# kevinh-e/BetaOne

Hardware: AMD Instinct MI355X
Metric: mcts_nodes_per_sec (higher is better)
Workload: dtype f32 (3 x f16 split, f32 accumulate)

## Files before the change

betaone_amd/csrc/bo_engine.cpp:

```cpp
#include "../../include/betaone_engine.h"
#include "../../include/betaone_lab.h"

#include "bo_tree.h"
#include "bo_fastw.h"
#include "bo_select_wide.h"
#include "bo_replay.h"
#include "bo_train.h"
#include "bo_metrics.h"
#include "bo_pgn.h"
#include "bo_san.h"
#include "bo_analyse.h"
#include "bo_reanalyse.h"
#include "bo_perft.h"
#include "bo_mate.h"
#include "bo_book.h"
#include "bo_merge.h"
#include "bo_tb.h"
#include "bo_nn_fused.h"
#include "bo_conv.h"
#include "bo_tower.h"
#include "bo_tower_wg.h"
#include "bo_tower_h.h"
#include "bo_tower_s.h"
#include "bo_tower_s16.h"
// ... 31 lines not shown
    int sel_profile = 0, sel_pending = 0;
    long long sel_launches = 0;
    double sel_ms = 0.0;
#if !defined(BO_WAVE_EMU)
    hipEvent_t sel_ev0 = nullptr, sel_ev1 = nullptr;
#endif
    bool fast = false;
    bo_config cfg;
    int device;
    std::vector<void *> allocs;
    int *d_go = nullptr, *d_action = nullptr;
    std::vector<int> h_i32;
    std::vector<HostRng> rng;
    int *d_res_blk = nullptr, *d_info_blk = nullptr;
    int *h_res = nullptr, *h_info = nullptr;
    int watch_seen = 0;
    double *h_noise = nullptr;
    int *h_go = nullptr;
    int *h_action = nullptr;
    int action_flip = 0;
    rt_event ev_action[2]{};
    bool ev_action_made[2] = {false, false};
    bool ship = true;
    bool prefetch_valid = false;
    std::vector<int> h_nl, h_term;
    bool nl_valid = false;
    void *setup_dev = nullptr, *setup_host = nullptr;
    size_t setup_cap = 0;
    std::vector<unsigned char> noise_pending;
    std::vector<int> lazy_want;
    bool begin_lazy = false, ev_begin_made = false;
    rt_event ev_begin{};
    double *h_turn_u = nullptr;
    int *h_turn_flags = nullptr;
    double *d_turn_pw = nullptr;
    std::vector<double> turn_pw_host;
    double turn_pw_tfinal = 0.0;
    int *d_turn_action = nullptr, *d_turn_state = nullptr, *d_turn_cres = nullptr;
    float *d_turn_rv = nullptr;
    int *d_turn_resigned = nullptr, *d_turn_rnext = nullptr;
    std::vector<int> resign_en;
    float resign_t = 0.0f;
    int resign_k = 1;
    float *d_root_value = nullptr;
    TbTable *d_tb_tabs = nullptr;
    std::vector<int> turn_want;
// ... 146 lines not shown
    int **iscal[] = {&d.sims_done, &d.n_nodes, &d.rows, &d.n_runs, &d.n_ul, &d.req_nlegal, &d.status,
                     &d.trk_n, &d.n_hist, &d.ctx_mode, &d.root_nch, &d.stat_evals,
                     &d.stat_flushes, &d.stat_term_sims, &d.stat_levels, &d.stat_children_scanned, &e->d_go, &e->d_action};
    for (int **p : iscal) rc |= e->alloc(p, G);
    const size_t res_ints = G * (4 + 2 * (size_t)BO_RES_CAP) + 4, info_ints = G * 18;
    rc |= e->alloc(&e->d_res_blk, res_ints); rc |= e->alloc(&e->d_info_blk, info_ints);
    if (!rc) {
        d.res_n = e->d_res_blk; d.res_best_idx = e->d_res_blk + G; d.res_best_mv = e->d_res_blk + 2 * G; d.res_total = e->d_res_blk + 3 * G;
        d.res_idx = e->d_res_blk + 4 * G; d.res_val = reinterpret_cast<float *>(e->d_res_blk + 4 * G + G * BO_RES_CAP);
        d.res_watch = e->d_res_blk + G * (4 + 2 * (size_t)BO_RES_CAP); d.watch = nullptr; d.watch_n = 1;
        d.phase = e->d_info_blk; d.req_node = e->d_info_blk + G; d.root_nlegal = e->d_info_blk + 2 * G; d.root_term = e->d_info_blk + 3 * G;
        d.ply = e->d_info_blk + 4 * G;
        e->d_turn_action = e->d_info_blk + 5 * G; e->d_turn_state = e->d_info_blk + 6 * G; e->d_turn_cres = e->d_info_blk + 7 * G;
        e->d_turn_rv = reinterpret_cast<float *>(e->d_info_blk + 15 * G); e->d_turn_resigned = e->d_info_blk + 16 * G;
        e->d_turn_rnext = e->d_info_blk + 17 * G;
        rt_memset(e->d_res_blk, 0, res_ints * 4, nullptr); rt_memset(e->d_info_blk, 0, info_ints * 4, nullptr);
    }
    rc |= rt_host_alloc((void **)&e->h_res, res_ints * 4); rc |= rt_host_alloc((void **)&e->h_info, info_ints * 4);
    rc |= rt_host_alloc((void **)&e->h_noise, G * BO_MAX_MOVES * sizeof(double)); rc |= rt_host_alloc((void **)&e->h_go, G * 4);
    rc |= rt_host_alloc((void **)&e->h_action, 2 * G * 4);
    rc |= rt_host_alloc((void **)&e->h_turn_u, G * sizeof(double)); rc |= rt_host_alloc((void **)&e->h_turn_flags, G * 4);
    rc |= e->alloc(&e->d_turn_pw, (size_t)cfg->num_simulations + 1);
    { const char *v = getenv("BETAONE_TURN_COPIES"); e->ship = !(v && v[0] == '1'); }
    rc |= e->alloc(&d.gpos, G * c.PLY_CAP); rc |= e->alloc(&d.trk, G * c.TRK_CAP); rc |= e->alloc(&d.trk_cnt, G * c.TRK_CAP);
    rc |= e->alloc(&d.hist, G * 7);
    rc |= e->alloc(&d.n_visits, N); rc |= e->alloc(&d.parent, N); rc |= e->alloc(&d.first_child, N); rc |= e->alloc(&d.n_children, N);
    rc |= e->alloc(&d.q, N); rc |= e->alloc(&d.prior, N); rc |= e->alloc(&d.move, N); rc |= e->alloc(&d.term, N);
    rc |= e->alloc(&d.eval_slot, N); rc |= e->alloc(&d.npos, N);
    rc |= e->alloc(&d.run_leaf, G * c.B); rc |= e->alloc(&d.run_cnt, G * c.B);
    rc |= e->alloc(&d.ul_node, G * c.UL_MAX); rc |= e->alloc(&d.ul_nlegal, G * c.UL_MAX); rc |= e->alloc(&d.ul_value, G * c.UL_MAX);
    rc |= e->alloc(&d.ul_move, G * c.UL_MAX * BO_CH_CAP); rc |= e->alloc(&d.ul_prior, G * c.UL_MAX * BO_CH_CAP);
    rc |= e->alloc(&d.req_moves, G * BO_MAX_MOVES); rc |= e->alloc(&d.root_moves, G * BO_MAX_MOVES);
    rc |= e->alloc(&d.root_child_rank, G * 2 * BO_CH_CAP); rc |= e->alloc(&d.noise, G * BO_MAX_MOVES);
    rc |= e->alloc(&d.played, G * c.PLY_CAP);
    rc |= e->alloc(&d.prof, G * BO_PROF_SLOTS);
    rc |= e->alloc(&d.resign_cnt, 2 * G); rc |= e->alloc(&e->d_root_value, G);
    if (!rc) rt_memset(d.resign_cnt, 0, 2 * G * 4, nullptr);
    rc |= e->alloc(&e->d_tb_tabs, (size_t)TB_MAX_TABLES); rc |= e->alloc(&d.tb_stat, 3 * G);
    if (!rc) rt_memset(d.tb_stat, 0, 3 * G * 4, nullptr);
    d.tb_tabs = e->d_tb_tabs; d.tb_n = 0; d.tb_flags = 0;
    d.played_now = nullptr;
    if (fast) {
        FastW &f = e->f;
        const size_t L = (size_t)cfg->leaves_per_step;
        f.L = (int)L;
        f.sel_ut = 2; f.sel_flags = FW_SEL_OCT;
// ... 248 lines not shown
    e->prefetch_valid = false;
    if (e->fast) {
        const int rows = e->d.c.G * e->f.L;
        if (policy_kind != BO_POLICY_NONE) RT(RT_LAUNCH(bo_k_fw_apply, rows, stream, e->d, e->f, policy_dev, policy_kind));
#if !defined(BO_WAVE_EMU)
        if (e->sel_profile) {
            if (!e->sel_ev0) { RT((int)hipEventCreate(&e->sel_ev0)); RT((int)hipEventCreate(&e->sel_ev1)); }
            if (e->sel_pending) {
                float ms = 0.0f;
                RT((int)hipEventSynchronize(e->sel_ev1));
                RT((int)hipEventElapsedTime(&ms, e->sel_ev0, e->sel_ev1));
                e->sel_ms += ms; e->sel_launches++; e->sel_pending = 0;
            }
            RT((int)hipEventRecord(e->sel_ev0, (hipStream_t)stream));
        }
#endif
        RT(launch_fw_select(e, value_dev, policy_kind, stream));
#if !defined(BO_WAVE_EMU)
        if (e->sel_profile) { RT((int)hipEventRecord(e->sel_ev1, (hipStream_t)stream)); e->sel_pending = 1; }
#endif
        RT(RT_LAUNCH(bo_k_fw_leaf, rows, stream, e->d, e->f, nn_in_dev));
    } else {
        if (e->d.tb_n > 0 && (e->d.tb_flags & TBF_SEARCH)) RT(RT_LAUNCH(bo_k_step_tb, e->d.c.G, stream, e->d, policy_dev, value_dev, policy_kind, nn_in_dev, vt));
        else RT(RT_LAUNCH(bo_k_step, e->d.c.G, stream, e->d, policy_dev, value_dev, policy_kind, nn_in_dev, vt));
    }
    return BO_OK;
}
extern "C" int bo_step(bo_engine *e, const float *policy_dev, const float *value_dev, int policy_kind, float *nn_in_dev,
                       void *stream) {
    if (!e || !nn_in_dev) return fail(BO_E_ARG, "null argument");
    if (policy_kind != BO_POLICY_NONE && (!policy_dev || !value_dev)) return fail(BO_E_ARG, "policy/value required");
    return step_launch(e, policy_dev, value_dev, policy_kind, nn_in_dev, stream, StepTail{nullptr, nullptr, nullptr, nullptr, 0});
}
extern "C" int bo_step_heads(bo_engine *e, const float *logits_dev, const float *vpart_dev, const float *b1_dev, const float *w2_dev,
                             const float *b2_dev, int rows, float *nn_in_dev, void *stream) {
    if (!e || !nn_in_dev || !logits_dev || !vpart_dev || !b1_dev || !w2_dev || !b2_dev) return fail(BO_E_ARG, "null argument");
    if (e->fast) return fail(BO_E_CONFIG, "bo_step_heads: the reference-semantics search only (fast mode evaluates rows, not games)");
    if (rows < e->d.c.G) return fail(BO_E_ARG, "bo_step_heads: the partial sums must hold a row per game (rows >= G)");
    return step_launch(e, logits_dev, nullptr, BO_POLICY_LOGITS, nn_in_dev, stream, StepTail{vpart_dev, b1_dev, w2_dev, b2_dev, rows});
}

extern "C" int bo_search_poll(bo_engine *e, int32_t *n_running, int32_t *n_requested, int32_t *requested_mask, void *stream) {
    if (!e) return fail(BO_E_ARG, "null engine");
    const size_t G = (size_t)e->d.c.G;
    RT(rt_d2h(e->h_info, e->d_info_blk, 2 * G * 4, stream));
    const int *ph = e->h_info, *rq = e->h_info + G;
    RT(rt_sync(stream));
// ... 382 lines not shown
        RT(rt_h2d(e->d_turn_pw, e->turn_pw_host.data(), ((size_t)S + 1) * sizeof(double), stream));
        RT(rt_sync(stream));
        e->turn_pw_tfinal = t_final;
    }
    if (!redo) {
        for (int g = 0; g < G; g++) {
            const double temp = move_number[g] < threshold ? t_initial : t_final;
            int fl = (active[g] ? 1 : 0) | (want_next[g] ? 4 : 0);
            if (active[g] && !(fabs(temp - 1.0) < 1e-6)) fl |= 2;
            if (active[g] && (int)e->resign_en.size() == G && e->resign_en[g]) fl |= 8;
            e->h_turn_flags[g] = fl;
            if (active[g]) e->h_turn_u[g] = hr_double(&e->rng[g]);
        }
        e->turn_want.assign(want_next, want_next + G);
    }
    TurnArgs a;
    a.u = e->h_turn_u; a.flags = e->h_turn_flags; a.pw = e->d_turn_pw;
    a.action = e->d_turn_action; a.state = e->d_turn_state; a.cres = e->d_turn_cres;
    a.root_value = e->d_turn_rv; a.resigned = e->d_turn_resigned; a.resign_next = e->d_turn_rnext;
    a.resign_t = e->resign_t; a.resign_k = e->resign_k;
    e->prefetch_valid = false;
    e->nl_valid = false;
    RT(RT_LAUNCH(bo_k_turn_sample, G, stream, e->d, a));
    RT(RT_LAUNCH(bo_k_turn_play, G, stream, e->d, a, nn_in_dev));
    const size_t Gs = (size_t)G, watch_off = Gs * (4 + 2 * (size_t)BO_RES_CAP);
    int rc = ship(e, e->h_info + 2 * Gs, (const int *)e->d_info_blk + 2 * Gs, 15 * Gs, e->h_res + watch_off, (const int *)e->d_res_blk + watch_off, 4, stream);
    if (rc) return rc;
    if (!e->ev_turn_made) { RT(rt_event_create(&e->ev_turn)); e->ev_turn_made = true; }
    RT(rt_event_record(e->ev_turn, stream));
    rc = bo_step(e, nullptr, nullptr, BO_POLICY_NONE, nn_in_dev, stream);
    if (rc) return rc;
    e->turn_outstanding = true;
    return BO_OK;
}

extern "C" int bo_selfplay_autoturn_ready(bo_engine *e, int32_t *ready_out) {
    if (!e || !ready_out) return fail(BO_E_ARG, "null argument");
    if (!e->turn_outstanding) return fail(BO_E_STATE, "no bo_selfplay_autoturn outstanding");
#if defined(BO_WAVE_EMU)
    *ready_out = 1;
#else
    const hipError_t q = hipEventQuery(e->ev_turn);
    if (q != hipSuccess && q != hipErrorNotReady) return fail(BO_E_HIP, std::string("hipEventQuery: ") + hipGetErrorString(q));
    *ready_out = q == hipSuccess ? 1 : 0;
#endif
    return BO_OK;
}

extern "C" int bo_selfplay_autoturn_collect_ex(bo_engine *e, int32_t *res_n, int32_t *res_idx, float *res_val, int32_t *best_idx,
                                               int32_t *action_out, int32_t *n_legal_out, int32_t *terminal_out, int32_t *go_out,
                                               float *root_value_out, int32_t *resigned_out, int32_t *completed) {
    if (!e || !res_n || !res_idx || !res_val || !action_out || !completed) return fail(BO_E_ARG, "null argument");
    if (!e->turn_outstanding) return fail(BO_E_STATE, "no bo_selfplay_autoturn outstanding");
    RT(rt_event_sync(e->ev_turn));
// ... 1710 lines not shown
    return BO_OK;
#endif
}

extern "C" int bo_nn_heads(const void *p_dev, const void *v_dev, const float *wp_dev, const float *bp_dev, const float *w1_dev,
                           const float *b1_dev, const float *w2_dev, const float *b2_dev, float *policy_out_dev, float *value_out_dev,
                           float *scratch_dev, int batch, int flags, void *stream) {
#if defined(BO_WAVE_EMU)
    (void)p_dev; (void)v_dev; (void)wp_dev; (void)bp_dev; (void)w1_dev; (void)b1_dev; (void)w2_dev; (void)b2_dev; (void)policy_out_dev;
    (void)value_out_dev; (void)scratch_dev; (void)batch; (void)flags; (void)stream;
    return fail(BO_E_CONFIG, "bo_nn_heads is a gfx950-only kernel");
#else
    if (!p_dev || !v_dev || !wp_dev || !bp_dev || !w1_dev || !b1_dev || !w2_dev || !b2_dev || !policy_out_dev || (!value_out_dev && !(flags & 4)) || !scratch_dev)
        return fail(BO_E_ARG, "null argument");
    if ((flags & 4) && (flags & 1)) return fail(BO_E_ARG, "bo_nn_heads: flags 4 (no rows kernel) leaves LOGITS: it excludes flags 1 (softmax)");
    if (batch < 1 || batch > 65536) return fail(BO_E_ARG, "bo_nn_heads: 1 <= batch <= 65536");
    bo_heads_args a;
    a.p = p_dev; a.v = v_dev; a.wp = wp_dev; a.bp = bp_dev; a.w1 = w1_dev; a.b1 = b1_dev; a.w2 = w2_dev; a.b2 = b2_dev;
    a.policy_out = policy_out_dev; a.value_out = value_out_dev;
    a.vpart = scratch_dev;
    a.B = batch; a.softmax = flags & 1; a.pb = bo_heads_policy_boards(batch);
    const int otw = 4 / (a.pb >> 5);
    const unsigned tiles = (unsigned)(((batch + a.pb - 1) / a.pb) * ((BO_HEADS_NA / 32 + otw - 1) / otw) + ((batch + 63) / 64) * 4 * BO_HEADS_KS);
    if (flags & 2) hipLaunchKernelGGL(bo_k_heads_tiles<true>, dim3(tiles), dim3(256), 0, (hipStream_t)stream, a, bo_heads_pair{});
    else hipLaunchKernelGGL(bo_k_heads_tiles<false>, dim3(tiles), dim3(256), 0, (hipStream_t)stream, a, bo_heads_pair{});
    if (!(flags & 4)) hipLaunchKernelGGL(bo_k_heads_rows, dim3((unsigned)batch), dim3(256), 0, (hipStream_t)stream, a);
    RT((int)hipGetLastError());
    return BO_OK;
#endif
}

extern "C" int bo_nn_heads_pair(const void *p_dev, const void *v_dev, const bo_head_weights *net0, const bo_head_weights *net1,
                                const int32_t *sel_dev, float *policy_out_dev, float *value_out_dev, float *scratch_dev, int batch, int flags,
                                void *stream) {
#if defined(BO_WAVE_EMU)
    (void)p_dev; (void)v_dev; (void)net0; (void)net1; (void)sel_dev; (void)policy_out_dev; (void)value_out_dev; (void)scratch_dev; (void)batch;
    (void)flags; (void)stream;
    return fail(BO_E_CONFIG, "bo_nn_heads_pair is a gfx950-only kernel");
#else
    if (!p_dev || !v_dev || !net0 || !net1 || !sel_dev || !policy_out_dev || !value_out_dev || !scratch_dev) return fail(BO_E_ARG, "null argument");
    for (const bo_head_weights *w : {net0, net1})
        if (!w->wp || !w->bp || !w->w1 || !w->b1 || !w->w2 || !w->b2) return fail(BO_E_ARG, "null head weight");
    if (flags & ~3) return fail(BO_E_ARG, "bo_nn_heads_pair: flags 1 (softmax) and 2 (fp16 planes) only");
    if (batch < 1 || batch > 65536) return fail(BO_E_ARG, "bo_nn_heads_pair: 1 <= batch <= 65536");
    bo_heads_args a;
    a.p = p_dev; a.v = v_dev; a.wp = net0->wp; a.bp = net0->bp; a.w1 = net0->w1; a.b1 = net0->b1; a.w2 = net0->w2; a.b2 = net0->b2;
    a.policy_out = policy_out_dev; a.value_out = value_out_dev;
// ... 941 lines not shown
```

betaone_amd/csrc/bo_heads.h:

```cpp
#pragma once
#if !defined(BO_WAVE_EMU)
#include <hip/hip_runtime.h>
#include "bo_tower.h"

#define BO_HEADS_NA 4672
#define BO_HEADS_KP 128
#define BO_HEADS_KV 2048
#define BO_HEADS_NH 256
#define BO_HEADS_KS 16
#define BO_HEADS_PITCH 132

struct bo_heads_args {
    const void *p, *v;
    const float *wp, *bp, *w1, *b1, *w2, *b2;
    float *policy_out, *value_out;
    float *vpart;
    int B, softmax;
    int pb;
};
static inline int bo_heads_policy_boards(int batch) { return batch > 64 ? 128 : batch > 32 ? 64 : 32; }

struct bo_heads_pair {
    const int32_t *sel = nullptr;
    const float *wp = nullptr, *bp = nullptr, *w1 = nullptr, *b1 = nullptr, *w2 = nullptr, *b2 = nullptr;
};

template <bool HALF>
__device__ __forceinline__ bo_f32x4 bo_heads_load4(const void *base, size_t e) {
    if constexpr (HALF) {
        typedef _Float16 h4 __attribute__((ext_vector_type(4)));
        const h4 h = *reinterpret_cast<const h4 *>(reinterpret_cast<const _Float16 *>(base) + e);
        return bo_f32x4{(float)h[0], (float)h[1], (float)h[2], (float)h[3]};
    } else {
        return *reinterpret_cast<const bo_f32x4 *>(reinterpret_cast<const float *>(base) + e);
    }
}

template <bool HALF, bool PAIR = false>
__global__ void __launch_bounds__(256)
bo_k_heads_tiles(bo_heads_args a, bo_heads_pair pr) {
    __shared__ __attribute__((aligned(16))) float tileA[64 * BO_HEADS_PITCH], tileW[64 * BO_HEADS_PITCH];
    const int tid = threadIdx.x, lane = tid & 63, wave = __builtin_amdgcn_readfirstlane(tid >> 6), kq = lane >> 4, i = lane & 15;
    const int B = a.B, pb = a.pb, nbw = pb >> 5, otw = 4 / nbw, NPT = (BO_HEADS_NA / 32 + otw - 1) / otw, n_policy = ((B + pb - 1) / pb) * NPT;
    const int wg = (int)blockIdx.x;
    if (wg < n_policy) {
        const int rb = wg / NPT, ct = wg - rb * NPT, r0 = pb * rb + 32 * (wave % nbw), c0 = 32 * (otw * ct + wave / nbw);
        if (c0 >= BO_HEADS_NA) return;
        bool has[2] = {true, false};
        if constexpr (PAIR) {
            const bool in = lane < 32 && r0 + lane < B;
            const int s1 = in ? (pr.sel[r0 + lane] != 0) : 0;
            has[0] = __ballot(in && !s1) != 0ull;
            has[1] = __ballot(in && s1) != 0ull;
        }
        for (int pass = 0; pass < (PAIR ? 2 : 1); pass++) {
            if (PAIR && !has[pass]) continue;
            const float *wp = PAIR && pass ? pr.wp : a.wp, *bp = PAIR && pass ? pr.bp : a.bp;
            const int only_net = PAIR && has[0] && has[1] ? pass : -1;
            const bo_f32x4 *w4 = reinterpret_cast<const bo_f32x4 *>(wp);
            constexpr int PG = BO_HEADS_KP / 16;
            bo_f32x4 fp[PG][2], fw[PG][2];
#pragma unroll
            for (int t = 0; t < PG; t++) {
                const int kk = 16 * t + 4 * kq;
#pragma unroll
                for (int c = 0; c < 2; c++) fw[t][c] = w4[((size_t)(c0 + 16 * c + i) * BO_HEADS_KP + kk) >> 2];
#pragma unroll
// ... 27 lines not shown
                    const int row = r0 + 16 * rt + i;
                    if (row < B && (only_net < 0 || (pr.sel[row] != 0) == only_net))
                        *reinterpret_cast<bo_f32x4 *>(a.policy_out + (size_t)row * BO_HEADS_NA + col) =
                            bo_f32x4{acc[c][rt][0] + bias[c][0], acc[c][rt][1] + bias[c][1], acc[c][rt][2] + bias[c][2], acc[c][rt][3] + bias[c][3]};
                }
            }
        }
    } else {
        const int vt = wg - n_policy, ks = vt & (BO_HEADS_KS - 1), ht = (vt >> 4) & 3, rbv = vt >> 6;
        const int r0 = 64 * rbv, h0 = 64 * ht, k0 = (BO_HEADS_KV / BO_HEADS_KS) * ks;
        bool has[2] = {true, false};
        if constexpr (PAIR) {
            const bool in = r0 + lane < B;
            const int s1 = in ? (pr.sel[r0 + lane] != 0) : 0;
            has[0] = __ballot(in && !s1) != 0ull;
            has[1] = __ballot(in && s1) != 0ull;
        }
        for (int pass = 0; pass < (PAIR ? 2 : 1); pass++) {
            if (PAIR && !has[pass]) continue;
            if (PAIR && pass && has[0]) __syncthreads();
            const float *w1 = PAIR && pass ? pr.w1 : a.w1;
            const int only_net = PAIR && has[0] && has[1] ? pass : -1;
            const bo_f32x4 *w4 = reinterpret_cast<const bo_f32x4 *>(w1);
            bo_f32x4 ga[8], gw[8];
#pragma unroll
            for (int q = 0; q < 8; q++) {
                const int idx = tid + 256 * q, row = idx >> 5, c4 = idx & 31;
                ga[q] = r0 + row < B ? bo_heads_load4<HALF>(a.v, ((size_t)(r0 + row)) * BO_HEADS_KV + k0 + 4 * c4) : bo_f32x4{0, 0, 0, 0};
                gw[q] = w4[(((size_t)(h0 + row)) * BO_HEADS_KV + k0) / 4 + c4];
            }
#pragma unroll
            for (int q = 0; q < 8; q++) {
                const int idx = tid + 256 * q, row = idx >> 5, c4 = idx & 31;
                *reinterpret_cast<bo_f32x4 *>(&tileA[row * BO_HEADS_PITCH + 4 * c4]) = ga[q];
                *reinterpret_cast<bo_f32x4 *>(&tileW[row * BO_HEADS_PITCH + 4 * c4]) = gw[q];
            }
            __syncthreads();
            const int hb = 32 * (wave & 1), bb = 32 * (wave >> 1);
            bo_f32x4 acc[2][2];
#pragma unroll
            for (int c = 0; c < 2; c++)
#pragma unroll
                for (int rt = 0; rt < 2; rt++) acc[c][rt] = bo_f32x4{0, 0, 0, 0};
#pragma unroll
            for (int t = 0; t < BO_HEADS_KV / BO_HEADS_KS / 16; t++) {
                bo_f32x4 fw[2], fv[2];
#pragma unroll
                for (int c = 0; c < 2; c++) fw[c] = *reinterpret_cast<const bo_f32x4 *>(&tileW[(hb + 16 * c + i) * BO_HEADS_PITCH + 16 * t + 4 * kq]);
#pragma unroll
                for (int rt = 0; rt < 2; rt++) fv[rt] = *reinterpret_cast<const bo_f32x4 *>(&tileA[(bb + 16 * rt + i) * BO_HEADS_PITCH + 16 * t + 4 * kq]);
#pragma unroll
                for (int e = 0; e < 4; e++)
#pragma unroll
                    for (int c = 0; c < 2; c++)
#pragma unroll
                        for (int rt = 0; rt < 2; rt++) acc[c][rt] = __builtin_amdgcn_mfma_f32_16x16x4f32(fw[c][e], fv[rt][e], acc[c][rt], 0, 0, 0);
            }
#pragma unroll
            for (int c = 0; c < 2; c++)
#pragma unroll
                for (int rt = 0; rt < 2; rt++) {
                    const int row = r0 + bb + 16 * rt + i;
                    if (row < B && (only_net < 0 || (pr.sel[row] != 0) == only_net))
                        *reinterpret_cast<bo_f32x4 *>(a.vpart + ((size_t)ks * B + row) * BO_HEADS_NH + h0 + hb + 16 * c + 4 * kq) = acc[c][rt];
                }
        }
    }
}

template <bool PAIR>
__device__ __forceinline__ void bo_heads_rows_body(const bo_heads_args &a, const bo_heads_pair &q) {
    __shared__ float sred[8];
    const int tid = threadIdx.x, lane = tid & 63, wave = __builtin_amdgcn_readfirstlane(tid >> 6);
    const int B = a.B, row = (int)blockIdx.x;
    const float *b1 = a.b1, *w2 = a.w2, *b2 = a.b2;
    if constexpr (PAIR) {
        if (__builtin_amdgcn_readfirstlane(q.sel[row]) != 0) { b1 = q.b1; w2 = q.w2; b2 = q.b2; }
    }
    float part[BO_HEADS_KS];
// ... 286 lines not shown
```

betaone_amd/csrc/bo_tree.h:

```cpp
#pragma once
#include "bo_chess.h"
#include "bo_tb_probe.h"
#include <math.h>

#define BO_CH_CAP 32
#define BO_PATH_CAP 1024
#define BO_RES_CAP 256
#define BO_PLANES 120
#ifndef BO_PROF_SLOTS
#define BO_PROF_SLOTS 16
#endif
#define BO_ROW (BO_PLANES * 64)

enum { PH_IDLE = 0, PH_RUN = 1, PH_DONE = 2 };
enum { ST_OK = 0, ST_NODE_OVERFLOW = 1, ST_DEPTH_OVERFLOW = 2, ST_NAN_SCORE = 4, ST_PLY_OVERFLOW = 8,
       ST_ILLEGAL_ACTION = 16, ST_UL_OVERFLOW = 32, ST_TRK_OVERFLOW = 64 };
enum { POLICY_NONE = 0, POLICY_LOGITS = 1, POLICY_PROBS = 2 };

struct EngCfg {
    int G, S, B;
    int NCAP, PLY_CAP, TRK_CAP;
    int nstride;
    int UL_MAX, CH_MAX;
    float cpuct, keep;
// ... 723 lines not shown
        for (int ks = 0; ks < 16; ks++) r.part[w][ks] = t.vpart[((size_t)ks * t.rows + g) * 256 + lane + 64 * w];
        r.b1[w] = t.b1[lane + 64 * w];
        r.w2[w] = t.w2[lane + 64 * w];
    }
    r.b2 = t.b2[0];
}
BO_DEV float tail_value(const TailRegs &r) {
    float s[4];
    BO_UNROLL
    for (int w = 0; w < 4; w++) {
        float h = 0.0f;
        BO_UNROLL
        for (int ks = 0; ks < 16; ks++) h += r.part[w][ks];
        h += r.b1[w];
        s[w] = (h > 0.0f ? h : 0.0f) * r.w2[w];
    }
    for (int m = 32; m >= 1; m >>= 1) {
        BO_UNROLL
        for (int w = 0; w < 4; w++) s[w] = s[w] + bo_shfl_xor_f(s[w], m);
    }
    return tanhf(((s[0] + s[1]) + (s[2] + s[3])) + r.b2);
}

BO_DEV void apply_leaf(const Eng &e, int g, int leaf, const float *row, int kind, const float *value_of, const StepTail &vt, StepShared &sh,
                       int *n_ul_io, int *flags) {
    const size_t no = NOFF(e, g);
    const int lane = bo_lane();
    const int n = e.req_nlegal[g];
    const bo_mv *mv = e.req_moves + (size_t)g * BO_MAX_MOVES;
    int slot = *n_ul_io;
    if (slot >= e.c.UL_MAX) { *flags |= ST_UL_OVERFLOW; slot = e.c.UL_MAX - 1; }
    const size_t uo = (size_t)g * e.c.UL_MAX + slot;
    float value;
    if (kind == POLICY_PROBS) {
        value = value_of[g];
        for (int j = lane; j < n; j += 64) sh.pv[j] = row[move_to_index(mv[j])];
    } else {
        float mx, sum;
        if (vt.vpart) {
            TailRegs tr;
            tail_load(vt, g, tr);
            row_max_sum(row, &mx, &sum);
            value = tail_value(tr);
        } else {
            value = value_of[g];
            row_max_sum(row, &mx, &sum);
        }
        for (int j = lane; j < n; j += 64) sh.pv[j] = bo_exp_row(row[move_to_index(mv[j])] - mx) / sum;
    }
    bo_sync();
    const int M = n < e.c.CH_MAX ? n : e.c.CH_MAX;
    for (int j = lane; j < n; j += 64) {
        int r = stable_rank(sh.pv, n, j);
        if (r < M) { e.ul_move[uo * BO_CH_CAP + r] = mv[j]; e.ul_prior[uo * BO_CH_CAP + r] = sh.pv[j]; }
    }
    if (lane == 0) {
        e.ul_node[uo] = leaf;
        e.ul_nlegal[uo] = n;
        e.ul_value[uo] = value;
        e.eval_slot[no + leaf] = (short)slot;
    }
    *n_ul_io = slot + 1;
    bo_sync();
}


BO_DEV float tb_leaf_value(int t, int kc) {
    const float m = 1.0f - (float)kc * (1.0f / 1024.0f);
    return t == TERM_TB_LOSS ? m : t == TERM_TB_WIN ? -m : 0.0f;
}
template <bool TB>
BO_DEV int step_body(const Eng &e, int g, const float *policy, const float *value, int kind, float *nn_in, StepShared &sh, const StepTail &vt) {
    const int lane = bo_lane();
    const size_t no = NOFF(e, g);
    int flags = 0;
    int sims = e.sims_done[g], rows = e.rows[g], n_runs = e.n_runs[g], n_ul = e.n_ul[g], n_nodes = e.n_nodes[g];
    int req = e.req_node[g];
    int *rl = e.run_leaf + (size_t)g * e.c.B, *rc = e.run_cnt + (size_t)g * e.c.B;
    float *row = nn_in + (size_t)g * BO_ROW;

    const bool prof = e.c.profile != 0;
    unsigned long long pc[8] = {0, 0, 0, 0, 0, 0, 0, 0};
    int n_iter = 0, n_first = 0, n_burst = 0, n_burst_sims = 0, n_general = 0, n_swaps = 0;
    unsigned long long tk = prof ? bo_clock() : 0ull;
    const unsigned long long t_start = tk;
#define BO_PROF(slot)                                                    \
    if (prof) { const unsigned long long _n = bo_clock(); pc[slot] += _n - tk; tk = _n; }
    if (req >= 0 && kind == POLICY_NONE) return n_nodes;
    const float *lut = e.sqrt_lut;
    if (req >= 0) {
        if (req == 0) apply_root(e, g, policy + (size_t)g * BO_NUM_ACTIONS, kind, sh, &n_nodes, &flags);
        else apply_leaf(e, g, req, policy + (size_t)g * BO_NUM_ACTIONS, kind, value, vt, sh, &n_ul, &flags);
        req = -1;
    }
    BO_PROF(0)
    int phase = PH_RUN;
    bool burst_tables_staged = false;
    int term_budget = e.c.B;
    int b_depth = 0;
    float b_tv = 0.0f;
    int path_leaf = -1, path_depth = -1;
    for (;;) {
        if (sims >= e.c.S) {
            if (rows > 0) { flush_pending(e, g, n_runs, n_ul, &n_nodes, sh.path2, &flags, path_leaf, sh.path, path_depth); rows = n_runs = n_ul = 0; }
            BO_PROF(5)
            phase = PH_DONE;
            break;
        }
        int depth;
        const int leaf = select_leaf(e, g, &flags, sh.path, &depth, lut);
        path_leaf = leaf; path_depth = depth;
        n_iter++;
        BO_PROF(1)
        int t = e.term[no + leaf];
        int tb_k = 0;
// ... 15 lines not shown
                    if (t != 0) {
                        tb_k = t == TERM_TB_DRAW ? 0 : k < 512 ? k : 512;
                        if (lane == 0) { e.eval_slot[no + leaf] = (short)tb_k; e.tb_stat[3 * g] += 1; }
                    }
                }
            }
            if (lane == 0) e.term[no + leaf] = (signed char)t;
            if (t == 0) {
                for (int j = lane; j < n; j += 64) e.req_moves[(size_t)g * BO_MAX_MOVES + j] = sh.moves[j];
                if (lane == 0) e.req_nlegal[g] = n;
            }
            bo_sync();
            BO_PROF(2)
        }
        if (t > 0) {
            float tv = t == 1 ? 1.0f : 0.0f;
            const bool tb_leaf = TB && t >= TERM_TB_WIN;
            if (tb_leaf) tv = tb_leaf_value(t, tb_k);
            int applied = 1;
            bool small = depth <= BO_BURST_LEVELS && BO_BURST_FITS(e.c.S);
            for (int k = 0; k < depth && small; k++) small = e.n_children[no + sh.path[k]] <= 16;
            BO_PROF(6)
            const int may = e.c.S - sims < term_budget ? e.c.S - sims : term_budget;
            if (small) {
                const bool small_b = b_depth > 0 && e.c.burst_two != 0;
                applied = terminal_burst<TB>(e, g, sh.path, depth, tv, may, sh.probs, &burst_tables_staged, sh.bpath, tb_leaf ? -1 : small_b ? b_depth : 0, b_tv,
                                             &n_swaps);
                n_burst++; n_burst_sims += applied;
                bo_sync();
                if (lane <= depth) sh.bpath[lane] = sh.path[lane];
                b_depth = tb_leaf ? 0 : depth; b_tv = tv;
                bo_sync();
            }
            else { backup_run(e, g, leaf, tv, 1, sh.path2, &flags, sh.path, depth); n_general++; }
            BO_PROF(7)
            sims += applied;
            term_budget -= applied;
            if (lane == 0) e.stat_term_sims[g] += applied;
            if (tb_leaf && lane == 0) e.tb_stat[3 * g + 1] += applied;
            BO_PROF(3)
            if (term_budget <= 0 && sims < e.c.S) break;
            continue;
        }
        if (e.eval_slot[no + leaf] < 0) {
            encode_leaf(e, g, row, e.npos[no + leaf]);
            req = leaf;
            if (lane == 0) e.stat_evals[g] += 1;
// ... 11 lines not shown
        BO_PROF(5)
    }
#undef BO_PROF
    if (prof && lane == 0) {
        const unsigned long long total = bo_clock() - t_start;
        if (e.c.profile == 1 || total > (unsigned long long)e.c.profile) {
            unsigned long long *pp = e.prof + (size_t)g * BO_PROF_SLOTS;
            pp[10] += (unsigned long long)n_burst; pp[11] += (unsigned long long)n_burst_sims; pp[12] += (unsigned long long)n_general;
            pp[13] += pc[6]; pp[14] += pc[7]; pp[15] += (unsigned long long)n_swaps;
            for (int i = 0; i < 6; i++) pp[i] += pc[i];
            pp[6] += total;
            pp[7] += 1;
            pp[8] += (unsigned long long)n_iter;
            pp[9] += (unsigned long long)n_first;
        }
    }
    if (lane == 0) {
        e.sims_done[g] = sims; e.rows[g] = rows; e.n_runs[g] = n_runs; e.n_ul[g] = n_ul; e.n_nodes[g] = n_nodes;
        e.req_node[g] = req; e.phase[g] = phase;
        if (flags) e.status[g] |= flags;
    }
    return n_nodes;
}
BO_KERNEL void bo_k_step(Eng e, const float *policy, const float *value, int kind, float *nn_in, StepTail vt) {
    BO_SHARED StepShared sh;
    const int g = bo_block();
    if (e.phase[g] != PH_RUN) return;
    step_body<false>(e, g, policy, value, kind, nn_in, sh, vt);
}
BO_KERNEL void bo_k_step_tb(Eng e, const float *policy, const float *value, int kind, float *nn_in, StepTail vt) {
    BO_SHARED StepShared sh;
    const int g = bo_block();
    if (e.phase[g] != PH_RUN) return;
    step_body<true>(e, g, policy, value, kind, nn_in, sh, vt);
}

BO_DEV int root_prepare(const Eng &e, int g, StepShared &sh) {
    const size_t no = NOFF(e, g);
    const int lane = bo_lane();
    const int ply = e.ply[g];
    const DPos P = e.gpos[(size_t)g * e.c.PLY_CAP + ply];
    if (lane == 0) {
        init_node(e, no, 0, -1, 1.0f, 0, P);
        e.n_nodes[g] = 1; e.sims_done[g] = 0; e.rows[g] = 0; e.n_runs[g] = 0; e.n_ul[g] = 0;
        e.req_node[g] = -1; e.phase[g] = PH_IDLE; e.root_nch[g] = 0;
        if (e.ctx_mode[g] == 0) {
            int nh = ply < 7 ? ply : 7;
            e.n_hist[g] = nh;
            for (int i = 0; i < nh; i++) e.hist[(size_t)g * 7 + i] = e.gpos[(size_t)g * e.c.PLY_CAP + ply - nh + i];
        }
    }
    bo_sync();
    bool chk;
    const int n = bo_movegen(P, sh.moves, &chk);
    if (lane == 0) sh.path[0] = 0;
    bo_sync();
    int t = terminal_eval(e, g, sh.path, 0, P, sh.moves, n, chk, sh.moves2, sh.chain);
// ... 274 lines not shown
        n = bo_popc64(nz);
        if (n >= 1) { const int l0 = bo_lsb64(nz); ia = bo_shfl(idx, l0); ca = bo_shfl(v, l0); }
        if (n >= 2) { const int l1 = bo_lsb64(nz & (nz - 1)); ib = bo_shfl(idx, l1); cb = bo_shfl(v, l1); }
        bool ok;
        act = turn_sample(n, ia, ca, ib, cb, total, e.c.S, (fl & 2) != 0, a.pw, a.u[g], &ok);
        if (!ok) { st = 2; act = -1; }
        rv = e.q[no];
        if (fl & 8) {
            const int cnt = e.resign_cnt[2 * g + (e.ply[g] & 1)];
            rnext = rv < a.resign_t ? cnt + 1 : 0;
            if (st == 0 && rnext >= a.resign_k) { rsg = 1; act = -1; }
        }
    }
    if (lane == 0) {
        a.root_value[g] = rv; a.resigned[g] = rsg; a.resign_next[g] = rnext;
        a.action[g] = act; a.state[g] = st;
        int *c = a.cres + (size_t)g * 8;
        c[0] = n; c[1] = e.res_best_idx[g]; c[2] = e.res_best_mv[g]; c[3] = total; c[4] = ia; c[5] = ib;
        c[6] = n >= 1 ? __builtin_bit_cast(int, (float)((double)ca / (double)total)) : 0;
        c[7] = n >= 2 ? __builtin_bit_cast(int, (float)((double)cb / (double)total)) : 0;
    }
}

BO_KERNEL void bo_k_turn_play(Eng e, TurnArgs a, float *nn_in) {
    BO_SHARED StepShared sh;
    const int g = bo_block(), lane = bo_lane();
    bool bad = false;
    for (int j0 = 0; j0 < e.c.G; j0 += 64) bad = bad || bo_ballot(j0 + lane < e.c.G && a.state[j0 + lane] != 0) != 0;
    if (bad) return;
    if (lane == 0 && a.resign_next[g] >= 0) e.resign_cnt[2 * g + (e.ply[g] & 1)] = a.resign_next[g];
    if (a.resigned[g]) return;
    int t = play_body(e, g, a.action[g], sh);
    if (t < 0) t = e.root_term[g];
    if (!(a.flags[g] & 4) || t != 0) return;
    encode_static(e, g, nn_in + (size_t)g * BO_ROW);
    if (lane == 0) e.phase[g] = PH_RUN;
}

BO_KERNEL void bo_k_root_value(Eng e, float *out) {
    const int g = bo_block() * 64 + bo_lane();
    if (g < e.c.G) out[g] = e.q[NOFF(e, g)];
}

BO_KERNEL void bo_k_encode_game(Eng e, int g, int first, float *out) {
    const int i = first + bo_block(), s = bo_lane();
    const DPos *gp = e.gpos + (size_t)g * e.c.PLY_CAP;
    float *row = out + (size_t)bo_block() * BO_ROW;
    const int h0 = i - 7 > 0 ? i - 7 : 0, nb = i + 1 - h0;
    for (int pl = 0; pl < (8 - nb) * 14; pl++) row[pl * 64 + s] = 0.0f;
    for (int k = 0; k < nb; k++) {
        DPos H = gp[h0 + k];
        encode_block(row, 8 - nb + k, H, tracker_reps(e, g, H));
    }
    encode_scalars(row, gp[i]);
}

BO_KERNEL void bo_k_encode_positions(const DPos *pos, int n_pos, int first, float *out) {
    const int i = first + bo_block(), s = bo_lane();
    float *row = out + (size_t)bo_block() * BO_ROW;
// ... 22 lines not shown
```

Before: 80.86 million.

## Fuse turn play, host ship and step; add lean step kernel and split-K value tiles

Adds a lean bo_k_step variant with the value-tail and profiling code compiled out, used when those features are off. Fuses the turn play kernel with the copy of info and watch data to host memory and the following step, removing separate launches and copies. The value-head tiles now load K in two halves, halving the shared tiles and register staging, behind an env toggle. This adds code paths with different host-visible write ordering, which may affect when the host sees the copied data.

New measurement: 81.91 million, median of 6. 1.3% higher.

```diff
diff --git a/betaone_amd/csrc/bo_engine.cpp b/betaone_amd/csrc/bo_engine.cpp
--- a/betaone_amd/csrc/bo_engine.cpp
+++ b/betaone_amd/csrc/bo_engine.cpp
@@ -77,6 +77,8 @@
     rt_event ev_action[2]{};
     bool ev_action_made[2] = {false, false};
     bool ship = true;
+    bool turn_fused = true;
+    bool step_lean = true;
     bool prefetch_valid = false;
     std::vector<int> h_nl, h_term;
     bool nl_valid = false;
@@ -269,6 +271,8 @@
     rc |= rt_host_alloc((void **)&e->h_turn_u, G * sizeof(double)); rc |= rt_host_alloc((void **)&e->h_turn_flags, G * 4);
     rc |= e->alloc(&e->d_turn_pw, (size_t)cfg->num_simulations + 1);
     { const char *v = getenv("BETAONE_TURN_COPIES"); e->ship = !(v && v[0] == '1'); }
+    { const char *v = getenv("BETAONE_STEP_LEAN"); e->step_lean = !(v && v[0] == '0'); }
+    { const char *v = getenv("BETAONE_TURN_FUSED"); e->turn_fused = !(v && v[0] == '0'); }
     rc |= e->alloc(&d.gpos, G * c.PLY_CAP); rc |= e->alloc(&d.trk, G * c.TRK_CAP); rc |= e->alloc(&d.trk_cnt, G * c.TRK_CAP);
     rc |= e->alloc(&d.hist, G * 7);
     rc |= e->alloc(&d.n_visits, N); rc |= e->alloc(&d.parent, N); rc |= e->alloc(&d.first_child, N); rc |= e->alloc(&d.n_children, N);
@@ -563,7 +567,8 @@
         RT(RT_LAUNCH(bo_k_fw_leaf, rows, stream, e->d, e->f, nn_in_dev));
     } else {
         if (e->d.tb_n > 0 && (e->d.tb_flags & TBF_SEARCH)) RT(RT_LAUNCH(bo_k_step_tb, e->d.c.G, stream, e->d, policy_dev, value_dev, policy_kind, nn_in_dev, vt));
-        else RT(RT_LAUNCH(bo_k_step, e->d.c.G, stream, e->d, policy_dev, value_dev, policy_kind, nn_in_dev, vt));
+        else if (e->step_lean && !vt.vpart && !e->d.c.profile) RT(RT_LAUNCH(bo_k_step, e->d.c.G, stream, e->d, policy_dev, value_dev, policy_kind, nn_in_dev));
+        else RT(RT_LAUNCH(bo_k_step_opt, e->d.c.G, stream, e->d, policy_dev, value_dev, policy_kind, nn_in_dev, vt));
     }
     return BO_OK;
 }
@@ -992,14 +997,26 @@
     e->prefetch_valid = false;
     e->nl_valid = false;
     RT(RT_LAUNCH(bo_k_turn_sample, G, stream, e->d, a));
-    RT(RT_LAUNCH(bo_k_turn_play, G, stream, e->d, a, nn_in_dev));
     const size_t Gs = (size_t)G, watch_off = Gs * (4 + 2 * (size_t)BO_RES_CAP);
-    int rc = ship(e, e->h_info + 2 * Gs, (const int *)e->d_info_blk + 2 * Gs, 15 * Gs, e->h_res + watch_off, (const int *)e->d_res_blk + watch_off, 4, stream);
+    int rc = BO_OK;
+    const bool step_in_turn = e->turn_fused && e->step_lean && !e->d.c.profile && !(e->d.tb_n > 0 && (e->d.tb_flags & TBF_SEARCH));
+    if (e->turn_fused) {
+        TurnShip s;
+        s.step = step_in_turn ? 1 : 0;
+        s.info_dst = e->h_info + 2 * Gs; s.info_src = (const int *)e->d_info_blk + 2 * Gs;
+        s.watch_dst = e->h_res + watch_off; s.watch_src = (const int *)e->d_res_blk + watch_off;
+        RT(RT_LAUNCH(bo_k_turn_play_ship, G, stream, e->d, a, nn_in_dev, s));
+    } else {
+        RT(RT_LAUNCH(bo_k_turn_play, G, stream, e->d, a, nn_in_dev));
+        rc = ship(e, e->h_info + 2 * Gs, (const int *)e->d_info_blk + 2 * Gs, 15 * Gs, e->h_res + watch_off, (const int *)e->d_res_blk + watch_off, 4, stream);
+    }
     if (rc) return rc;
     if (!e->ev_turn_made) { RT(rt_event_create(&e->ev_turn)); e->ev_turn_made = true; }
     RT(rt_event_record(e->ev_turn, stream));
-    rc = bo_step(e, nullptr, nullptr, BO_POLICY_NONE, nn_in_dev, stream);
-    if (rc) return rc;
+    if (!step_in_turn) {
+        rc = bo_step(e, nullptr, nullptr, BO_POLICY_NONE, nn_in_dev, stream);
+        if (rc) return rc;
+    }
     e->turn_outstanding = true;
     return BO_OK;
 }
@@ -2756,7 +2773,10 @@
     a.B = batch; a.softmax = flags & 1; a.pb = bo_heads_policy_boards(batch);
     const int otw = 4 / (a.pb >> 5);
     const unsigned tiles = (unsigned)(((batch + a.pb - 1) / a.pb) * ((BO_HEADS_NA / 32 + otw - 1) / otw) + ((batch + 63) / 64) * 4 * BO_HEADS_KS);
+    const char *orv = getenv("BETAONE_HEADS_ONE_ROUND");
+    const bool one_round = !(orv && orv[0] == '0');
     if (flags & 2) hipLaunchKernelGGL(bo_k_heads_tiles<true>, dim3(tiles), dim3(256), 0, (hipStream_t)stream, a, bo_heads_pair{});
+    else if (one_round) hipLaunchKernelGGL((bo_k_heads_tiles<false, false, true>), dim3(tiles), dim3(256), 0, (hipStream_t)stream, a, bo_heads_pair{});
     else hipLaunchKernelGGL(bo_k_heads_tiles<false>, dim3(tiles), dim3(256), 0, (hipStream_t)stream, a, bo_heads_pair{});
     if (!(flags & 4)) hipLaunchKernelGGL(bo_k_heads_rows, dim3((unsigned)batch), dim3(256), 0, (hipStream_t)stream, a);
     RT((int)hipGetLastError());
diff --git a/betaone_amd/csrc/bo_heads.h b/betaone_amd/csrc/bo_heads.h
--- a/betaone_amd/csrc/bo_heads.h
+++ b/betaone_amd/csrc/bo_heads.h
@@ -36,13 +36,17 @@
     }
 }
 
-template <bool HALF, bool PAIR = false>
+template <bool HALF, bool PAIR = false, bool ONE_ROUND = false>
 __global__ void __launch_bounds__(256)
 bo_k_heads_tiles(bo_heads_args a, bo_heads_pair pr) {
-    __shared__ __attribute__((aligned(16))) float tileA[64 * BO_HEADS_PITCH], tileW[64 * BO_HEADS_PITCH];
+    static_assert(!(ONE_ROUND && PAIR), "the two-net launch keeps whole-K value tiles");
+    constexpr int VKH = ONE_ROUND ? 2 : 1, VK = BO_HEADS_KV / BO_HEADS_KS / VKH, VPITCH = VK + 4;
+    static_assert(ONE_ROUND || VPITCH == BO_HEADS_PITCH, "whole-K tiles keep BO_HEADS_PITCH");
+    __shared__ __attribute__((aligned(16))) float tileA[64 * VPITCH], tileW[64 * VPITCH];
     const int tid = threadIdx.x, lane = tid & 63, wave = __builtin_amdgcn_readfirstlane(tid >> 6), kq = lane >> 4, i = lane & 15;
     const int B = a.B, pb = a.pb, nbw = pb >> 5, otw = 4 / nbw, NPT = (BO_HEADS_NA / 32 + otw - 1) / otw, n_policy = ((B + pb - 1) / pb) * NPT;
-    const int wg = (int)blockIdx.x;
+    const int n_value = (int)gridDim.x - n_policy;
+    const int wg = ONE_ROUND ? ((int)blockIdx.x < n_value ? n_policy + (int)blockIdx.x : (int)blockIdx.x - n_value) : (int)blockIdx.x;
     if (wg < n_policy) {
         const int rb = wg / NPT, ct = wg - rb * NPT, r0 = pb * rb + 32 * (wave % nbw), c0 = 32 * (otw * ct + wave / nbw);
         if (c0 >= BO_HEADS_NA) return;
@@ -116,20 +120,16 @@
             const float *w1 = PAIR && pass ? pr.w1 : a.w1;
             const int only_net = PAIR && has[0] && has[1] ? pass : -1;
             const bo_f32x4 *w4 = reinterpret_cast<const bo_f32x4 *>(w1);
-            bo_f32x4 ga[8], gw[8];
-#pragma unroll
-            for (int q = 0; q < 8; q++) {
-                const int idx = tid + 256 * q, row = idx >> 5, c4 = idx & 31;
-                ga[q] = r0 + row < B ? bo_heads_load4<HALF>(a.v, ((size_t)(r0 + row)) * BO_HEADS_KV + k0 + 4 * c4) : bo_f32x4{0, 0, 0, 0};
-                gw[q] = w4[(((size_t)(h0 + row)) * BO_HEADS_KV + k0) / 4 + c4];
-            }
-#pragma unroll
-            for (int q = 0; q < 8; q++) {
-                const int idx = tid + 256 * q, row = idx >> 5, c4 = idx & 31;
-                *reinterpret_cast<bo_f32x4 *>(&tileA[row * BO_HEADS_PITCH + 4 * c4]) = ga[q];
-                *reinterpret_cast<bo_f32x4 *>(&tileW[row * BO_HEADS_PITCH + 4 * c4]) = gw[q];
-            }
-            __syncthreads();
+            constexpr int LPR = VK / 4, NQ = 8 / VKH;
+            bo_f32x4 ga[VKH][NQ], gw[VKH][NQ];
+#pragma unroll
+            for (int h = 0; h < VKH; h++)
+#pragma unroll
+                for (int q = 0; q < NQ; q++) {
+                    const int idx = tid + 256 * q, row = idx / LPR, c4 = idx % LPR;
+                    ga[h][q] = r0 + row < B ? bo_heads_load4<HALF>(a.v, ((size_t)(r0 + row)) * BO_HEADS_KV + k0 + VK * h + 4 * c4) : bo_f32x4{0, 0, 0, 0};
+                    gw[h][q] = w4[(((size_t)(h0 + row)) * BO_HEADS_KV + k0 + VK * h) / 4 + c4];
+                }
             const int hb = 32 * (wave & 1), bb = 32 * (wave >> 1);
             bo_f32x4 acc[2][2];
 #pragma unroll
@@ -137,18 +137,29 @@
 #pragma unroll
                 for (int rt = 0; rt < 2; rt++) acc[c][rt] = bo_f32x4{0, 0, 0, 0};
 #pragma unroll
-            for (int t = 0; t < BO_HEADS_KV / BO_HEADS_KS / 16; t++) {
-                bo_f32x4 fw[2], fv[2];
-#pragma unroll
-                for (int c = 0; c < 2; c++) fw[c] = *reinterpret_cast<const bo_f32x4 *>(&tileW[(hb + 16 * c + i) * BO_HEADS_PITCH + 16 * t + 4 * kq]);
-#pragma unroll
-                for (int rt = 0; rt < 2; rt++) fv[rt] = *reinterpret_cast<const bo_f32x4 *>(&tileA[(bb + 16 * rt + i) * BO_HEADS_PITCH + 16 * t + 4 * kq]);
-#pragma unroll
-                for (int e = 0; e < 4; e++)
-#pragma unroll
-                    for (int c = 0; c < 2; c++)
-#pragma unroll
-                        for (int rt = 0; rt < 2; rt++) acc[c][rt] = __builtin_amdgcn_mfma_f32_16x16x4f32(fw[c][e], fv[rt][e], acc[c][rt], 0, 0, 0);
+            for (int h = 0; h < VKH; h++) {
+                if (h) __syncthreads();
+#pragma unroll
+                for (int q = 0; q < NQ; q++) {
+                    const int idx = tid + 256 * q, row = idx / LPR, c4 = idx % LPR;
+                    *reinterpret_cast<bo_f32x4 *>(&tileA[row * VPITCH + 4 * c4]) = ga[h][q];
+                    *reinterpret_cast<bo_f32x4 *>(&tileW[row * VPITCH + 4 * c4]) = gw[h][q];
+                }
+                __syncthreads();
+#pragma unroll
+                for (int t = 0; t < VK / 16; t++) {
+                    bo_f32x4 fw[2], fv[2];
+#pragma unroll
+                    for (int c = 0; c < 2; c++) fw[c] = *reinterpret_cast<const bo_f32x4 *>(&tileW[(hb + 16 * c + i) * VPITCH + 16 * t + 4 * kq]);
+#pragma unroll
+                    for (int rt = 0; rt < 2; rt++) fv[rt] = *reinterpret_cast<const bo_f32x4 *>(&tileA[(bb + 16 * rt + i) * VPITCH + 16 * t + 4 * kq]);
+#pragma unroll
+                    for (int e = 0; e < 4; e++)
+#pragma unroll
+                        for (int c = 0; c < 2; c++)
+#pragma unroll
+                            for (int rt = 0; rt < 2; rt++) acc[c][rt] = __builtin_amdgcn_mfma_f32_16x16x4f32(fw[c][e], fv[rt][e], acc[c][rt], 0, 0, 0);
+                }
             }
 #pragma unroll
             for (int c = 0; c < 2; c++)
diff --git a/betaone_amd/csrc/bo_tree.h b/betaone_amd/csrc/bo_tree.h
--- a/betaone_amd/csrc/bo_tree.h
+++ b/betaone_amd/csrc/bo_tree.h
@@ -769,6 +769,7 @@
     return tanhf(((s[0] + s[1]) + (s[2] + s[3])) + r.b2);
 }
 
+template <bool TAIL>
 BO_DEV void apply_leaf(const Eng &e, int g, int leaf, const float *row, int kind, const float *value_of, const StepTail &vt, StepShared &sh,
                        int *n_ul_io, int *flags) {
     const size_t no = NOFF(e, g);
@@ -784,7 +785,7 @@
         for (int j = lane; j < n; j += 64) sh.pv[j] = row[move_to_index(mv[j])];
     } else {
         float mx, sum;
-        if (vt.vpart) {
+        if (TAIL && vt.vpart) {
             TailRegs tr;
             tail_load(vt, g, tr);
             row_max_sum(row, &mx, &sum);
@@ -816,7 +817,7 @@
     const float m = 1.0f - (float)kc * (1.0f / 1024.0f);
     return t == TERM_TB_LOSS ? m : t == TERM_TB_WIN ? -m : 0.0f;
 }
-template <bool TB>
+template <bool TB, bool TAIL, bool PROF>
 BO_DEV int step_body(const Eng &e, int g, const float *policy, const float *value, int kind, float *nn_in, StepShared &sh, const StepTail &vt) {
     const int lane = bo_lane();
     const size_t no = NOFF(e, g);
@@ -826,7 +827,7 @@
     int *rl = e.run_leaf + (size_t)g * e.c.B, *rc = e.run_cnt + (size_t)g * e.c.B;
     float *row = nn_in + (size_t)g * BO_ROW;
 
-    const bool prof = e.c.profile != 0;
+    const bool prof = PROF && e.c.profile != 0;
     unsigned long long pc[8] = {0, 0, 0, 0, 0, 0, 0, 0};
     int n_iter = 0, n_first = 0, n_burst = 0, n_burst_sims = 0, n_general = 0, n_swaps = 0;
     unsigned long long tk = prof ? bo_clock() : 0ull;
@@ -837,7 +838,7 @@
     const float *lut = e.sqrt_lut;
     if (req >= 0) {
         if (req == 0) apply_root(e, g, policy + (size_t)g * BO_NUM_ACTIONS, kind, sh, &n_nodes, &flags);
-        else apply_leaf(e, g, req, policy + (size_t)g * BO_NUM_ACTIONS, kind, value, vt, sh, &n_ul, &flags);
+        else apply_leaf<TAIL>(e, g, req, policy + (size_t)g * BO_NUM_ACTIONS, kind, value, vt, sh, &n_ul, &flags);
         req = -1;
     }
     BO_PROF(0)
@@ -899,7 +900,7 @@
             for (int k = 0; k < depth && small; k++) small = e.n_children[no + sh.path[k]] <= 16;
             BO_PROF(6)
             const int may = e.c.S - sims < term_budget ? e.c.S - sims : term_budget;
-            if (small) {
+            if (__builtin_expect(small, 1)) {
                 const bool small_b = b_depth > 0 && e.c.burst_two != 0;
                 applied = terminal_burst<TB>(e, g, sh.path, depth, tv, may, sh.probs, &burst_tables_staged, sh.bpath, tb_leaf ? -1 : small_b ? b_depth : 0, b_tv,
                                              &n_swaps);
@@ -957,17 +958,23 @@
     }
     return n_nodes;
 }
-BO_KERNEL void bo_k_step(Eng e, const float *policy, const float *value, int kind, float *nn_in, StepTail vt) {
+BO_KERNEL void bo_k_step(Eng e, const float *policy, const float *value, int kind, float *nn_in) {
     BO_SHARED StepShared sh;
     const int g = bo_block();
     if (e.phase[g] != PH_RUN) return;
-    step_body<false>(e, g, policy, value, kind, nn_in, sh, vt);
+    step_body<false, false, false>(e, g, policy, value, kind, nn_in, sh, StepTail{nullptr, nullptr, nullptr, nullptr, 0});
+}
+BO_KERNEL void bo_k_step_opt(Eng e, const float *policy, const float *value, int kind, float *nn_in, StepTail vt) {
+    BO_SHARED StepShared sh;
+    const int g = bo_block();
+    if (e.phase[g] != PH_RUN) return;
+    step_body<false, true, true>(e, g, policy, value, kind, nn_in, sh, vt);
 }
 BO_KERNEL void bo_k_step_tb(Eng e, const float *policy, const float *value, int kind, float *nn_in, StepTail vt) {
     BO_SHARED StepShared sh;
     const int g = bo_block();
     if (e.phase[g] != PH_RUN) return;
-    step_body<true>(e, g, policy, value, kind, nn_in, sh, vt);
+    step_body<true, true, true>(e, g, policy, value, kind, nn_in, sh, vt);
 }
 
 BO_DEV int root_prepare(const Eng &e, int g, StepShared &sh) {
@@ -1288,9 +1295,8 @@
     }
 }
 
-BO_KERNEL void bo_k_turn_play(Eng e, TurnArgs a, float *nn_in) {
-    BO_SHARED StepShared sh;
-    const int g = bo_block(), lane = bo_lane();
+BO_DEV void turn_play_body(const Eng &e, const TurnArgs &a, float *nn_in, int g, StepShared &sh) {
+    const int lane = bo_lane();
     bool bad = false;
     for (int j0 = 0; j0 < e.c.G; j0 += 64) bad = bad || bo_ballot(j0 + lane < e.c.G && a.state[j0 + lane] != 0) != 0;
     if (bad) return;
@@ -1301,6 +1307,28 @@
     if (!(a.flags[g] & 4) || t != 0) return;
     encode_static(e, g, nn_in + (size_t)g * BO_ROW);
     if (lane == 0) e.phase[g] = PH_RUN;
+}
+BO_KERNEL void bo_k_turn_play(Eng e, TurnArgs a, float *nn_in) {
+    BO_SHARED StepShared sh;
+    turn_play_body(e, a, nn_in, bo_block(), sh);
+}
+
+struct TurnShip {
+    int *info_dst; const int *info_src;
+    int *watch_dst; const int *watch_src;
+    int step;
+};
+BO_KERNEL void bo_k_turn_play_ship(Eng e, TurnArgs a, float *nn_in, TurnShip s) {
+    BO_SHARED StepShared sh;
+    const int g = bo_block(), lane = bo_lane(), G = e.c.G;
+    turn_play_body(e, a, nn_in, g, sh);
+    bo_sync();
+    if (lane < 15) {
+        const size_t off = (lane < 5 || lane >= 13) ? (size_t)lane * G + g : (size_t)5 * G + (size_t)8 * g + (lane - 5);
+        s.info_dst[off] = s.info_src[off];
+    } else if (g == 0 && lane < 19) s.watch_dst[lane - 15] = s.watch_src[lane - 15];
+    if (!s.step || e.phase[g] != PH_RUN) return;
+    step_body<false, false, false>(e, g, nullptr, nullptr, POLICY_NONE, nn_in, sh, StepTail{nullptr, nullptr, nullptr, nullptr, 0});
 }
 
 BO_KERNEL void bo_k_root_value(Eng e, float *out) {
```
